# KyleHuang9/YOLO-LP

Measured on AMD Instinct MI355X. Metric: images/sec (640×640) end-to-end detect+NMS, yololps, 1/2/4/8 MI355X, higher is better.
Workload: dtype f16; 1 GPU; yololps 640x640 bs=32/GPU f16, synthetic frames resident in HBM, seeded random-init weights (sigma 0.25), conf 0.40 iou 0.45 max_det 1000; global_batch=32, parallelism=dp1: images sharded, all-gather of detections

## Files before the change

yolo-lp_amd/csrc/lp_conv3x3_pipe.inc:

```
#pragma once
#include "lp_conv_kernel.inc"
#include <type_traits>
#include <utility>

namespace lp {

template <int P> struct PipeCfg;
template <> struct PipeCfg<PIPE_D> { static constexpr int CB = 128, WC = 2, WP = 2, WGC = 2, WGP = 4, HPMAX = 384; };
template <> struct PipeCfg<PIPE_B> { static constexpr int CB = 64, WC = 2, WP = 2, WGC = 1, WGP = 8, HPMAX = 704; };
template <> struct PipeCfg<PIPE_F> { static constexpr int CB = 128, WC = 1, WP = 2, WGC = 4, WGP = 2, HPMAX = 384; };

template <> struct PipeCfg<PIPE_C> { static constexpr int CB = 32, WC = 1, WP = 2, WGC = 1, WGP = 8, HPMAX = 736; };

constexpr int PIPE_MAXC = 1024;
constexpr int PIPE_MAXCHUNKS = 64;

#ifndef LP_PIPE_ABL
#define LP_PIPE_ABL 0
#endif

template <typename F, int... I> __device__ __forceinline__ void static_for_impl(F&& f, std::integer_sequence<int, I...>) {
    (f(std::integral_constant<int, I>{}), ...);
}
template <int N, typename F> __device__ __forceinline__ void static_for(F&& f) {
// ... 192 lines not shown
            const unsigned long long p = (unsigned long long)a.src[sidx].ptr;
            c.tab[0] = (unsigned)p; c.tab[1] = (unsigned)(p >> 32);
            c.tab[2] = (unsigned)a.src[sidx].cs; c.tab[3] = (unsigned)((dq - a.chunk_begin[sidx]) * KC);
            c.ws = wts + ((long long)dma.ct * nchunks + dq) * (9 * CB * KC * 2);
        };
        auto halo_pieces = [&](const ChunkSrc& cc, char* buf) {
#pragma unroll
            for (int k = KH0; k < NPW; ++k) issue_piece(k, cc, buf, 1);
        };
        auto weight_pieces = [&](const ChunkSrc& cc, char* buf) {
#pragma unroll
            for (int k = 0; k < NPW; ++k) issue_piece(k, cc, buf, 2);
        };
        ChunkSrc c, c1;
        chunk_src_direct(c);
        if constexpr (LP_PRO_ORDER == 0) {
            halo_pieces(c, smem);
            dma_ok = dma_advance();
            if (dma_ok) {
                chunk_src_direct(c1);
                halo_pieces(c1, smem + SLOT);
            }
            weight_pieces(c, smem);
            if (dma_ok) weight_pieces(c1, smem + SLOT);
        } else {
            weight_pieces(c, smem);
            halo_pieces(c, smem);
            dma_ok = dma_advance();
            if (dma_ok) {
                chunk_src_direct(c1);
                weight_pieces(c1, smem + SLOT);
                halo_pieces(c1, smem + SLOT);
            }
        }
        if (dma_ok) dma_ok = dma_advance();
#ifdef LP_STAMPS
        st_p2 = __builtin_amdgcn_s_memtime();
#endif
        for (int i = tid; i < a.nct * CB; i += 512) bias_lds[i] = a.bias[i];
        if (tid < nchunks) {
            int sidx = 0;
#pragma unroll
            for (int k = 1; k < LP_MAX_SRC; ++k)
                if (k < a.nsrc && tid >= a.chunk_begin[k]) sidx = k;
            ChunkTab e;
            e.sp = (const T*)a.src[sidx].ptr;
            e.cs = a.src[sidx].cs;
            e.c0 = (tid - a.chunk_begin[sidx]) * KC;
            ctab[tid] = e;
// ... 296 lines not shown
```

yolo-lp_amd/csrc/lp_conv3x3_pipe16.inc:

```
#pragma once
#include "lp_conv3x3_pipe.inc"

namespace lp {

typedef float f32x4v __attribute__((ext_vector_type(4)));

template <typename T> struct Mma16;
template <> struct Mma16<f16> {
    static __device__ __forceinline__ f32x4v mma(f16x8 a, f16x8 b, f32x4v c) { return __builtin_amdgcn_mfma_f32_16x16x32_f16(a, b, c, 0, 0, 0); }
};
template <> struct Mma16<bf16> {
    static __device__ __forceinline__ f32x4v mma(bf16x8 a, bf16x8 b, f32x4v c) { return __builtin_amdgcn_mfma_f32_16x16x32_bf16(a, b, c, 0, 0, 0); }
};

template <int P> struct Pipe16Cfg;
template <> struct Pipe16Cfg<PIPE16_D> { static constexpr int CB = 128, WCB = 4, WPB = 4, WGC = 2, WGP = 4, HPMAX = 384; };
template <> struct Pipe16Cfg<PIPE16_F> { static constexpr int CB = 128, WCB = 2, WPB = 4, WGC = 4, WGP = 2, HPMAX = 384; };

__host__ __device__ __forceinline__ constexpr int quad_order(int i) { return ((i >> 2) == 2 ? 12 : (i >> 2) == 3 ? 8 : (i & 12)) + (i & 3); }

template <typename T, int P, bool DUAL = false>
__global__ __launch_bounds__(512) void conv3x3_pipe16_kernel(const ConvArgs a, const int total) {
    typedef Pipe16Cfg<P> C;
    typedef typename Mma<T>::V V;
    static_assert(sizeof(T) == 2, "16-bit activations only");
    constexpr int CB = C::CB, WCB = C::WCB, WPB = C::WPB, WGC = C::WGC, WGP = C::WGP, HPMAX = C::HPMAX;
    constexpr int NW = 8, ROWB = 32, KC = 16, EPG = 8;
    constexpr int NWP = 9 * CB / 32;
    constexpr int NHP = HPMAX / 32;
    static_assert((NWP + NHP) % NW == 0, "every wave must issue the same number of DMA instructions per chunk");
    constexpr int NPW = (NWP + NHP) / NW;
    constexpr int KH0 = NWP / NW;
    constexpr int NHK = NPW - KH0;
    constexpr int WOFF = HPMAX * ROWB;
    constexpr int SLOT = (HPMAX + 9 * CB) * ROWB;
    static_assert(WGC * WGP == NW, "8 waves");
    static_assert(WPB % 2 == 0, "the epilogue pairs pixel blocks");
    __shared__ __attribute__((aligned(1024))) char smem[3 * SLOT + PIPE_MAXC * 4 + PIPE_MAXCHUNKS * 16];
    float* const bias_lds = (float*)(smem + 3 * SLOT);
    const unsigned smem_lds = (unsigned)(size_t)(lds_char_t*)smem;

    const int tid = threadIdx.x;
    const int lane = tid & 63, wave = __builtin_amdgcn_readfirstlane(tid >> 6);
    const int li = lane & 15, g = lane >> 4;
    const int wvc = wave % WGC, wvp = wave / WGC;
    const int G = gridDim.x;

    const int tpi = a.tiles_y * a.tiles_x;
    const int npt = a.B * tpi;
    const int HH = a.TH + 2, HW = a.TW + 2, HP = a.hpitch;
    const int npix = a.TH * a.TW;
    const int nchunks = a.chunk_begin[a.nsrc];

    int hyx[NHK], hgc[NHK];
#pragma unroll
    for (int kk = 0; kk < NHK; ++kk) {
        const int j = (KH0 + kk) * NW + wave - NWP;
        const int slot = j * 64 + lane;
        const int hp = slot >> 1;
// ... 34 lines not shown
        o.b = pt / tpi;
        const int trem = pt - o.b * tpi;
        o.ty0 = (trem / a.tiles_x) * a.TH;
        o.tx0 = (trem % a.tiles_x) * a.TW;
        return true;
    };
    auto next_tile = [&](Tile& o) -> bool {
        int t = o.t;
        while (true) {
            t += G;
            if (decode(t, o)) return true;
            if (t >= total) return false;
        }
    };

    Tile dma, cmp;
    bool dma_ok = decode(blockIdx.x, dma) || next_tile(dma);
    if (!dma_ok) return;
    cmp = dma;
    int dq = 0;
    int hpix[NHK];
    auto dma_maps = [&]() {
#pragma unroll
        for (int kk = 0; kk < NHK; ++kk) {
            const int hy = hyx[kk] >> 16, hx = hyx[kk] & 0xffff;
            const int iy = dma.ty0 - 1 + hy, ix = dma.tx0 - 1 + hx;
            const bool ok = hyx[kk] >= 0 && iy >= 0 && iy < a.H && ix >= 0 && ix < a.W;
            hpix[kk] = ok ? (dma.b * a.H + iy) * a.W + ix : -1;
        }
    };
// ... 23 lines not shown
            const int cs = (int)cs_.tab[2];
            const int c = (int)cs_.tab[3] + hgc[kk];
            const T* const sp = (const T*)(((unsigned long long)cs_.tab[1] << 32) | cs_.tab[0]);
            const T* p = (hpix[kk] >= 0 && c < cs) ? sp + (long long)hpix[kk] * cs + c : zero;
            __builtin_amdgcn_global_load_lds((gbl_ptr_t)p, (lds_ptr_t)(buf + (i - NWP) * 1024), 16, 0, 0);
        }
    };
    auto dma_advance = [&]() {
        if (++dq < nchunks) return true;
        dq = 0;
        if (!next_tile(dma)) return false;
        dma_maps();
        return true;
    };

    {
        auto chunk_src_direct = [&](ChunkSrc& c) {
            int sidx = 0;
#pragma unroll
            for (int k = 1; k < LP_MAX_SRC; ++k)
                if (k < a.nsrc && dq >= a.chunk_begin[k]) sidx = k;
            const unsigned long long p = (unsigned long long)a.src[sidx].ptr;
            c.tab[0] = (unsigned)p; c.tab[1] = (unsigned)(p >> 32);
            c.tab[2] = (unsigned)a.src[sidx].cs; c.tab[3] = (unsigned)((dq - a.chunk_begin[sidx]) * KC);
            c.ws = wts + ((long long)dma.ct * nchunks + dq) * (9 * CB * KC * 2);
        };
        ChunkSrc c, c1;
        chunk_src_direct(c);
        dma_ok = dma_advance();
        chunk_src_direct(c1);
        auto halo_pieces = [&](const ChunkSrc& cc, char* buf) {
#pragma unroll
            for (int k = KH0; k < NPW; ++k) issue_piece(k, cc, buf, 1);
        };
        auto weight_pieces = [&](const ChunkSrc& cc, char* buf) {
#pragma unroll
            for (int k = 0; k < NPW; ++k) issue_piece(k, cc, buf, 2);
        };
        if constexpr (LP_PRO_ORDER == 0) {
            halo_pieces(c, smem); halo_pieces(c1, smem + SLOT); weight_pieces(c, smem); weight_pieces(c1, smem + SLOT);
        } else {
            weight_pieces(c, smem); weight_pieces(c1, smem + SLOT); halo_pieces(c, smem); halo_pieces(c1, smem + SLOT);
        }
        dma_ok = dma_advance();
        for (int i = tid; i < a.nct * CB; i += 512) bias_lds[i] = a.bias[i];
        if (tid < nchunks) {
            int sidx = 0;
#pragma unroll
            for (int k = 1; k < LP_MAX_SRC; ++k)
                if (k < a.nsrc && tid >= a.chunk_begin[k]) sidx = k;
            ChunkTab e;
            e.sp = (const T*)a.src[sidx].ptr;
            e.cs = a.src[sidx].cs;
            e.c0 = (tid - a.chunk_begin[sidx]) * KC;
            ctab[tid] = e;
        }
        asm volatile("s_waitcnt vmcnt(0)" ::: "memory");
    }
    __syncthreads();

    f32x4v acc[WCB][WPB];
    V fa[2][WCB], fb[2][WPB];
    int slot = 0;
    constexpr int NRD = WCB + WPB;
    auto read_one = [&](auto s_tag, int k, V(&af)[WCB], V(&bf)[WPB], unsigned va, unsigned vbb) {
        constexpr int s = decltype(s_tag)::value;
        constexpr int ta = s < 4 ? 2 * s : (s == 4 ? 8 : 2 * s - 9);
        constexpr int aimm = (s == 4 ? 0 : ta * CB * ROWB);
#pragma unroll
        for (int c = 0; c < WCB; ++c)
            if (k == c) LP_DS_READ128(af[c], va, aimm + c * 16 * ROWB);
#pragma unroll
        for (int p = 0; p < WPB; ++p)
            if (k == WCB + p) { const unsigned vb = vbb + boff[p][s]; LP_DS_READ128(bf[p], vb, 0); }
    };

    asm volatile("s_waitcnt lgkmcnt(0)" ::: "memory");
    __builtin_amdgcn_sched_barrier(0);
    {
        const unsigned va = smem_lds + aoffP;
#pragma unroll
        for (int k = 0; k < NRD; ++k) read_one(std::integral_constant<int, 0>{}, k, fa[0], fb[0], va, smem_lds);
    }
    constexpr int BE = 2, BO = 6;
    do {
#pragma unroll
        for (int c = 0; c < WCB; ++c) {
            const f32x4v bv = *(const f32x4v*)(bias_lds + cmp.ct * CB + (wvc * WCB + c) * 16 + (quad_order(4 * g)));
#pragma unroll
            for (int p = 0; p < WPB; ++p) acc[c][p] = bv;
        }
        asm volatile("s_waitcnt lgkmcnt(0)" ::: "memory");
        __builtin_amdgcn_sched_barrier(0);
        for (int cq = 0; cq < nchunks; cq += 4) {
            const int s0 = slot, s1 = slot == 2 ? 0 : slot + 1, s2 = slot == 0 ? 2 : slot - 1;
            const unsigned b0_ = smem_lds + (unsigned)s0 * SLOT, b1_ = smem_lds + (unsigned)s1 * SLOT, b2_ = smem_lds + (unsigned)s2 * SLOT;
            const unsigned vxa0 = (g < 2 ? b0_ + 8 * CB * ROWB : b1_) + aoffL, vxb0 = g < 2 ? b0_ : b1_;
            const unsigned vxa1 = (g < 2 ? b2_ + 8 * CB * ROWB : b0_) + aoffL, vxb1 = g < 2 ? b2_ : b0_;
            ChunkSrc nxt;
            static_for<18>([&](auto st_tag) {
                constexpr int S = decltype(st_tag)::value;
                constexpr int q = S / 9, st = S % 9;
                constexpr int cur = S & 1, nx = cur ^ 1;
                const unsigned bE = q == 0 ? b0_ : b2_, bO = q == 0 ? b1_ : b0_, bN = q == 0 ? b2_ : b1_;
                const int sE = q == 0 ? s0 : s2, sN = q == 0 ? s2 : s1;
                if constexpr (st == BE - 1 || st == BO - 1) chunk_src_request(nxt);
                if constexpr (st == BE || st == BO) {
                    asm volatile("s_waitcnt vmcnt(0)" ::: "memory");
                    __builtin_amdgcn_s_barrier();
                    asm volatile("" ::: "memory");
                    __builtin_amdgcn_sched_barrier(0);
                }
                if constexpr (st == BE || st == BO) asm volatile("s_waitcnt lgkmcnt(0)" : "+v"(nxt.tab)::"memory");
                else asm volatile("s_waitcnt lgkmcnt(0)" ::: "memory");
                __builtin_amdgcn_sched_barrier(0);
                constexpr int sn = (st + 1) % 9;
                const unsigned nva = sn == 4 ? (q == 0 ? vxa0 : vxa1) : ((st == 8 ? bN : (sn < 4 ? bE : bO)) + aoffP);
                const unsigned nvb = sn == 4 ? (q == 0 ? vxb0 : vxb1) : (st == 8 ? bN : (sn < 4 ? bE : bO));
                int nread = 0;
#pragma unroll
                for (int p = 0; p < WPB; ++p)
#pragma unroll
                    for (int c = 0; c < WCB; ++c) {
                        acc[c][p] = Mma16<T>::mma(fa[cur][c], fb[cur][p], acc[c][p]);
                        __builtin_amdgcn_sched_barrier(0);
                        if (nread < NRD) { read_one(std::integral_constant<int, sn>{}, nread, fa[nx], fb[nx], nva, nvb); ++nread; }
                        __builtin_amdgcn_sched_barrier(0);
                    }
                static_assert(NRD <= WCB * WPB, "one read per MFMA gap");
                if constexpr ((st >= BE && st < BE + 3) || (st >= BO && st < BO + 3)) {
                    constexpr int b0 = st >= BO ? BO : BE;
                    constexpr int k0 = (st - b0) * NPW / 3, k1 = (st - b0 + 1) * NPW / 3;
                    char* const nbuf = smem + (st >= BO ? sE : sN) * SLOT;
                    if (dma_ok) {
#pragma unroll
                        for (int k = k0; k < k1; ++k) issue_piece(k, nxt, nbuf);
                    }
                    __builtin_amdgcn_sched_barrier(0);
                    if constexpr (st == b0 + 2) { if (dma_ok) dma_ok = dma_advance(); }
                }
            });
            slot = s1;
        }

        {
            T* const out = (T*)a.out + (long long)cmp.b * a.out_img_stride;
            [[maybe_unused]] T* const out2 = DUAL ? (T*)a.out2 + (long long)cmp.b * a.out2_img_stride - a.out_split : nullptr;
            const T* const res = a.res ? (const T*)a.res + (long long)cmp.b * a.Ho * a.Wo * a.res_cs : nullptr;
            act_dispatch(a.act, [&](auto tag) {
                constexpr int ACT = decltype(tag)::value;
#pragma unroll
                for (int q = 0; q < WPB / 2; ++q) {
                    uint4 rv[WCB];
                    const int pl = (wvp * WPB + 2 * q + (g & 1)) * 16 + quad_order(li);
                    const int ty = (int)(((unsigned)pl * a.tw_magic) >> 22), tx = pl - ty * a.TW;
                    const int oy = cmp.ty0 + ty, ox = cmp.tx0 + tx;
                    const bool pok = pl < npix && oy < a.Ho && ox < a.Wo;
                    const long long opix = (long long)oy * a.Wo + ox;
// ... 27 lines not shown
                                const T* prr = (const T*)&rv[c];
#pragma unroll
                                for (int k = 0; k < EPG; ++k) pv[k] = from_f32<T>(to_f32(pv[k]) + a.alpha * to_f32(prr[k]));
                            }
                            if constexpr (DUAL) {
                                T* const dstp = cc >= a.out_split ? out2 + opix * a.out2_pix_stride + cc : out + opix * a.out_pix_stride + cc;
                                *(uint4*)dstp = v;
                            } else {
                                *(uint4*)(out + opix * a.out_pix_stride + cc) = v;
                            }
                        }
                    }
                }
            });
        }
    } while (next_tile(cmp));
    asm volatile("s_waitcnt lgkmcnt(0)" ::: "memory");
}

template <typename T, int P>
static inline int pipe16_launch_one(const ConvArgs& a, int ncu, hipStream_t st) {
    const int npt = a.B * a.tiles_y * a.tiles_x;
    const int total = a.nct * round_up(npt, 8);
    int grid = total < ncu ? total : ncu;
    if (a.out2) hipLaunchKernelGGL((conv3x3_pipe16_kernel<T, P, true>), dim3((unsigned)grid), dim3(512), 0, st, a, total);
    else hipLaunchKernelGGL((conv3x3_pipe16_kernel<T, P, false>), dim3((unsigned)grid), dim3(512), 0, st, a, total);
    hipError_t e = hipGetLastError();
    if (e != hipSuccess) return fail(LP_ERR_HIP, std::string("conv3x3 pipe16 launch: ") + hipGetErrorString(e));
    return LP_OK;
}

template <typename T>
// ... 10 lines not shown
```

yolo-lp_amd/csrc/lp_conv3x3_pipe16v.inc:

```
#pragma once
#include "lp_conv3x3_pipe16.inc"

namespace lp {

template <int P> struct Pipe16vCfg;
template <> struct Pipe16vCfg<PIPE16_V0> { static constexpr int CB = 128, WCB = 4, NBMAX = 7, WGC = 2, WGP = 4, HPMAX = 512; };
template <> struct Pipe16vCfg<PIPE16_V1> { static constexpr int CB = 128, WCB = 2, NBMAX = 7, WGC = 4, WGP = 2, HPMAX = 512; };

constexpr int PIPE16V_MAXC = 512;
constexpr int PIPE16V_MAXCHUNKS = 32;

template <typename T, int P, bool DUAL = false>
__global__ __launch_bounds__(512) void conv3x3_pipe16v_kernel(const ConvArgs a, const int total) {
    typedef Pipe16vCfg<P> C;
    typedef typename Mma<T>::V V;
    static_assert(sizeof(T) == 2, "16-bit activations only");
    constexpr int CB = C::CB, WCB = C::WCB, NBMAX = C::NBMAX, WGC = C::WGC, WGP = C::WGP, HPMAX = C::HPMAX;
    constexpr int NW = 8, ROWB = 32, KC = 16, EPG = 8;
    constexpr int NWP = 9 * CB / 32;
    constexpr int NHP = HPMAX / 32;
    constexpr int NPT = NWP + NHP;
    constexpr int NPW = (NPT + NW - 1) / NW;
    constexpr int KH0 = NWP / NW;
    constexpr int NHK = NPW - KH0;
    constexpr int WOFF = HPMAX * ROWB;
    constexpr int SLOT = (HPMAX + 9 * CB) * ROWB;
    static_assert(WGC * WGP == NW, "8 waves");
    static_assert(WCB <= NBMAX - 2, "the weight fragments of a K-step are requested in its first WCB blocks and must be older than the next step's first pixel fragment");
    static_assert(3 * SLOT + PIPE16V_MAXC * 4 + PIPE16V_MAXCHUNKS * 16 <= 160 * 1024, "LDS budget");
    static_assert(3 * (NBMAX / 2) >= NPW, "a piece round behind every odd block of the three steps after a barrier");
    __shared__ __attribute__((aligned(1024))) char smem[3 * SLOT + PIPE16V_MAXC * 4 + PIPE16V_MAXCHUNKS * 16];
    float* const bias_lds = (float*)(smem + 3 * SLOT);
    const unsigned smem_lds = (unsigned)(size_t)(lds_char_t*)smem;

    const int tid = threadIdx.x;
    const int lane = tid & 63, wave = __builtin_amdgcn_readfirstlane(tid >> 6);
    const int li = lane & 15, g = lane >> 4;
#ifdef LP_STAMPS
    const unsigned long long st_c0 = __builtin_amdgcn_s_memtime(), st_r0 = __builtin_amdgcn_s_memrealtime();
    unsigned long long st_p1 = 0, st_p2 = 0, st_p3 = 0, st_p4 = 0, st_loop = 0, st_epi = 0, st_last = 0;
#endif
    const int wvc = WGC == 2 ? (wave >> 2) : (wave & 3);
    const int wvp = WGC == 2 ? ((wave + 2 * (wave >> 2)) & 3) : (wave >> 2);
    const int G = gridDim.x;

    const int tpi = a.tiles_y * a.tiles_x;
    const int npt = a.B * tpi;
// ... 25 lines not shown
            int pl = (blk0 + p) * 16 + li;
            if (p >= nbw || pl >= npix) pl = 0;
            const int ty = (int)(((unsigned)pl * a.tw_magic) >> 22), tx = pl - ty * a.TW;
            bbase[p] = (ty * HP + tx) * ROWB + (g & 1) * 16;
        }
#pragma unroll
        for (int s = 0; s < 9; ++s) {
            const int ta = s < 4 ? 2 * s : (s == 4 ? 8 : 2 * s - 9);
            const int tb = s == 4 ? 0 : ta + 1;
            const int t = g < 2 ? ta : tb;
            voff[s] = ((t / 3) * HP + (t % 3)) * ROWB;
        }
        const int arow = (wvc * WCB) * 16 + quad_order(li);
        aoffL = WOFF + arow * ROWB + swz(arow, g & 1, 2) * 16;
        aoffP = aoffL + (g >> 1) * (CB * ROWB);
    };

    struct Tile { int t, ct, b, ty0, tx0; };
    auto decode = [&](int t, Tile& o) -> bool {
        o.t = t;
        if (t >= total) return false;
        const int jj = t >> 3;
        o.ct = jj % a.nct;
        const int pt = (jj / a.nct) * 8 + (t & 7);
        if (pt >= npt) return false;
        o.b = pt / tpi;
        const int trem = pt - o.b * tpi;
        o.ty0 = (trem / a.tiles_x) * a.TH;
        o.tx0 = (trem % a.tiles_x) * a.TW;
        return true;
// ... 62 lines not shown
#ifdef LP_P16V_DMAXH
#pragma unroll
            for (int r = 0; r < LP_P16V_DMAXH; ++r)
                __builtin_amdgcn_global_load_lds((gbl_ptr_t)p, (lds_ptr_t)(buf + (i - NWP) * 1024), 16, 0, 0);
#endif
        }
    };
    auto dma_advance = [&]() {
        if (++dq < nchunks) return true;
        dq = 0;
        if (!next_tile(dma)) return false;
        dma_maps();
        return true;
    };

    {
        auto chunk_src_direct = [&](ChunkSrc& c) {
            int sidx = 0;
#pragma unroll
            for (int k = 1; k < LP_MAX_SRC; ++k)
                if (k < a.nsrc && dq >= a.chunk_begin[k]) sidx = k;
            const unsigned long long p = (unsigned long long)a.src[sidx].ptr;
            c.tab[0] = (unsigned)p; c.tab[1] = (unsigned)(p >> 32);
            c.tab[2] = (unsigned)a.src[sidx].cs; c.tab[3] = (unsigned)((dq - a.chunk_begin[sidx]) * KC);
            c.ws = wts + ((long long)dma.ct * nchunks + dq) * (9 * CB * KC * 2);
        };
        ChunkSrc c, c1;
        chunk_src_direct(c);
        dma_ok = dma_advance();
        chunk_src_direct(c1);
        auto halo_pieces = [&](const ChunkSrc& cc, char* buf) {
#ifndef LP_P16V_PRO_SKIPH
#pragma unroll
            for (int k = KH0; k < NPW; ++k) issue_piece(k, cc, buf, 1);
#endif
        };
        auto weight_pieces = [&](const ChunkSrc& cc, char* buf) {
#ifndef LP_P16V_PRO_SKIPW
#pragma unroll
            for (int k = 0; k < NPW; ++k) issue_piece(k, cc, buf, 2);
#endif
        };
#ifndef LP_P16V_PRO_ORDER
#define LP_P16V_PRO_ORDER (LP_PRO_ORDER ? 3 : 0)
#endif
        if constexpr (LP_P16V_PRO_ORDER == 0) {
            halo_pieces(c, smem); halo_pieces(c1, smem + SLOT); weight_pieces(c, smem); weight_pieces(c1, smem + SLOT);
        } else if constexpr (LP_P16V_PRO_ORDER == 1) {
            halo_pieces(c, smem); weight_pieces(c, smem); weight_pieces(c1, smem + SLOT); halo_pieces(c1, smem + SLOT);
        } else if constexpr (LP_P16V_PRO_ORDER == 2) {
            weight_pieces(c, smem); halo_pieces(c, smem); weight_pieces(c1, smem + SLOT); halo_pieces(c1, smem + SLOT);
        } else if constexpr (LP_P16V_PRO_ORDER == 3) {
            weight_pieces(c, smem); weight_pieces(c1, smem + SLOT); halo_pieces(c, smem); halo_pieces(c1, smem + SLOT);
        } else {
            weight_pieces(c, smem); halo_pieces(c, smem); halo_pieces(c1, smem + SLOT); weight_pieces(c1, smem + SLOT);
        }
        dma_ok = dma_advance();
#ifdef LP_STAMPS
        st_p2 = __builtin_amdgcn_s_memtime();
#endif
        frag_maps();
        for (int i = tid; i < a.nct * CB; i += 512) bias_lds[i] = a.bias[i];
        if (tid < nchunks) {
            int sidx = 0;
#pragma unroll
            for (int k = 1; k < LP_MAX_SRC; ++k)
                if (k < a.nsrc && tid >= a.chunk_begin[k]) sidx = k;
            ChunkTab e;
            e.sp = (const T*)a.src[sidx].ptr;
            e.cs = a.src[sidx].cs;
            e.c0 = (tid - a.chunk_begin[sidx]) * KC;
            ctab[tid] = e;
        }
#ifdef LP_STAMPS
        st_p3 = __builtin_amdgcn_s_memtime();
#endif
        asm volatile("s_waitcnt vmcnt(0)" ::: "memory");
#ifdef LP_STAMPS
        st_p4 = __builtin_amdgcn_s_memtime();
#endif
    }
    __syncthreads();

    f32x4v acc[WCB][NBMAX];
    V fa[2][WCB];
    V fb[3];
    int slot = 0;
#ifndef LP_P16V_BE
#define LP_P16V_BE 2
#endif
#ifndef LP_P16V_BO
#define LP_P16V_BO 6
#endif
    constexpr int BE = LP_P16V_BE, BO = LP_P16V_BO;
    static_assert(BE >= 1 && BE <= 3 && BO >= 5 && BO <= 6, "barrier(e) in front of step 3's request of the cross step, barrier(o) behind step 4 with three steps of DMA issue left");
    constexpr int NBLK = 18 * NBMAX;

#ifdef LP_P16V_PRIO
    if (wave >= 4) __builtin_amdgcn_s_setprio(1);
#endif
    asm volatile("s_waitcnt lgkmcnt(0)" ::: "memory");
    __builtin_amdgcn_sched_barrier(0);
    {
        const unsigned va = smem_lds + aoffP;
#pragma unroll
        for (int c = 0; c < WCB; ++c) LP_DS_READ128(fa[0][c], va, c * 16 * ROWB);
        const unsigned vb0 = smem_lds + bbase[0] + voff[0], vb1 = smem_lds + bbase[1] + voff[0];
        LP_DS_READ128(fb[0], vb0, 0);
        LP_DS_READ128(fb[1], vb1, 0);
    }
#ifdef LP_STAMPS
    st_loop = __builtin_amdgcn_s_memtime();
#endif
    do {
#pragma unroll
        for (int c = 0; c < WCB; ++c) {
            const f32x4v bv = *(const f32x4v*)(bias_lds + cmp.ct * CB + (wvc * WCB + c) * 16 + (quad_order(4 * g)));
#pragma unroll
            for (int p = 0; p < NBMAX; ++p) acc[c][p] = bv;
        }
        asm volatile("s_waitcnt lgkmcnt(0)" ::: "memory");
        __builtin_amdgcn_sched_barrier(0);
        for (int cq = 0; cq < nchunks; cq += 4) {
            const int s0 = slot, s1 = slot == 2 ? 0 : slot + 1, s2 = slot == 0 ? 2 : slot - 1;
            const unsigned b0_ = smem_lds + (unsigned)s0 * SLOT, b1_ = smem_lds + (unsigned)s1 * SLOT, b2_ = smem_lds + (unsigned)s2 * SLOT;
            ChunkSrc nxt;
            static_for<18>([&](auto st_tag) {
                constexpr int S = decltype(st_tag)::value;
                constexpr int q = S / 9, st = S % 9;
                constexpr int cur = S & 1, nx = cur ^ 1;
                constexpr int sn = (st + 1) % 9;
                const unsigned bE = q == 0 ? b0_ : b2_, bO = q == 0 ? b1_ : b0_, bN = q == 0 ? b2_ : b1_;
                const int sE = q == 0 ? s0 : s2, sN = q == 0 ? s2 : s1;
                auto bstep = [&](int s, bool next_pair) -> unsigned {
                    const unsigned e = next_pair ? bN : bE, o = bO;
                    return (s < 4 ? e : (s == 4 ? (g < 2 ? e : o) : o)) + (unsigned)voff[s];
                };
                const unsigned vb_cur = bstep(st, false);
                const unsigned vb_nxt = bstep(sn, st == 8);
                const unsigned va_nxt = sn == 4 ? ((g < 2 ? bE + 8 * CB * ROWB : bO) + aoffL) : ((st == 8 ? bN : (sn < 4 ? bE : bO)) + aoffP);
                constexpr int ta_n = sn < 4 ? 2 * sn : (sn == 4 ? 8 : 2 * sn - 9);
                constexpr int aimm_n = sn == 4 ? 0 : ta_n * CB * ROWB;
                if constexpr (st == BE || st == BO) {
                    asm volatile("s_waitcnt vmcnt(0)" ::: "memory");
                    __builtin_amdgcn_s_barrier();
                    asm volatile("" ::: "memory");
                    __builtin_amdgcn_sched_barrier(0);
                }
#pragma unroll
                for (int p = 0; p < NBMAX; ++p) {
                    constexpr bool tab_step = (st == BE - 1 || st == BO - 1);
                    {
                        const int n = 1 + ((p >= 1 && p - 1 < WCB) ? 1 : 0) + ((tab_step && p == 1) ? 1 : 0);
                        if (n == 1) asm volatile("s_waitcnt lgkmcnt(1)" ::: "memory");
                        else if (n == 2) asm volatile("s_waitcnt lgkmcnt(2)" ::: "memory");
                        else asm volatile("s_waitcnt lgkmcnt(3)" ::: "memory");
                    }
                    __builtin_amdgcn_sched_barrier(0);
// ... 6 lines not shown
                            else if (e == 1) acc[c][p] = Mma16<T>::mma(fa[cur][c], fb[1], acc[c][p]);
                            else acc[c][p] = Mma16<T>::mma(fa[cur][c], fb[2], acc[c][p]);
                        }
                    }
                    __builtin_amdgcn_sched_barrier(0);
                    if (p < WCB) LP_DS_READ128(fa[nx][p], va_nxt, aimm_n + p * 16 * ROWB);
                    {
                        const int p2 = p + 2;
                        const unsigned vb = (p2 < NBMAX ? vb_cur + (unsigned)bbase[p2 < NBMAX ? p2 : 0] : vb_nxt + (unsigned)bbase[p2 < NBMAX ? 0 : p2 - NBMAX]);
                        const int e2 = (S * NBMAX + p + 2) % 3;
                        if (e2 == 0) LP_DS_READ128(fb[0], vb, 0);
                        else if (e2 == 1) LP_DS_READ128(fb[1], vb, 0);
                        else LP_DS_READ128(fb[2], vb, 0);
                    }
                    __builtin_amdgcn_sched_barrier(0);
                    if constexpr ((st >= BE && st < BE + 3) || (st >= BO && st < BO + 3)) {
                        constexpr int b0 = st >= BO ? BO : BE;
                        const int slotn = (st - b0) * (NBMAX / 2) + (p >> 1);
                        if ((p & 1) == 1 || p == NBMAX - 1) {
                            const int k = (p & 1) == 1 ? slotn : -1;
                            char* const nbuf = smem + (st >= BO ? sE : sN) * SLOT;
                            if (k >= 0 && k < NPW && dma_ok) issue_piece(k, nxt, nbuf);
                            __builtin_amdgcn_sched_barrier(0);
                        }
                        if (st == b0 + 2 && p == NBMAX - 1) { if (dma_ok) dma_ok = dma_advance(); }
                    }
                }
                if constexpr (st == BE || st == BO) asm volatile("" : "+v"(nxt.tab));
            });
            slot = s1;
        }
        (void)NBLK;

#ifdef LP_STAMPS
        const unsigned long long st_e0 = __builtin_amdgcn_s_memtime();
#endif
        {
            const long long torg = (long long)cmp.ty0 * a.Wo + cmp.tx0;
            const int cw = cmp.ct * CB + wvc * WCB * 16;
            T* const out = (T*)a.out + (long long)cmp.b * a.out_img_stride + torg * a.out_pix_stride + cw;
            [[maybe_unused]] T* const out2 = DUAL ? (T*)a.out2 + (long long)cmp.b * a.out2_img_stride + torg * a.out2_pix_stride + cw - a.out_split : nullptr;
            const T* const res = a.res ? (const T*)a.res + ((long long)cmp.b * a.Ho * a.Wo + torg) * a.res_cs + cw : nullptr;
            const int ylim = a.Ho - cmp.ty0, xlim = a.Wo - cmp.tx0;
            const int cg = (g >> 1) * 8;
            act_dispatch(a.act, [&](auto tag) {
                constexpr int ACT = decltype(tag)::value;
#pragma unroll
// ... 48 lines not shown
                                                                      : out + (unsigned)(erel[q] * a.out_pix_stride + c * 16 + cg);
                                    *(uint4*)dstp = v;
                                } else {
                                    *(uint4*)(out + (unsigned)(erel[q] * a.out_pix_stride + c * 16 + cg)) = v;
                                }
                            }
                        }
                    }
                }
            });
        }
#ifdef LP_STAMPS
        st_last = __builtin_amdgcn_s_memtime();
        st_epi += st_last - st_e0;
#endif
    } while (next_tile(cmp));
    asm volatile("s_waitcnt lgkmcnt(0)" ::: "memory");
#ifdef LP_STAMPS
    if (a.stamps && lane == 0) {
        unsigned long long* o = a.stamps + ((long long)(blockIdx.x * NW + wave)) * 8;
        asm volatile("s_waitcnt vmcnt(0)" ::: "memory");
        const unsigned long long st_end = __builtin_amdgcn_s_memtime();
        o[0] = st_end - st_c0; o[1] = __builtin_amdgcn_s_memrealtime() - st_r0;
        o[2] = st_loop - st_c0; o[3] = st_epi; o[4] = st_end - st_last; o[5] = o[0]; o[6] = nchunks; o[7] = 2;
        unsigned long long* o2 = a.stamps + (1 << 19) + ((long long)(blockIdx.x * NW + wave)) * 8;
        o2[0] = st_p1 - st_c0; o2[1] = st_p2 - st_p1; o2[2] = st_p3 - st_p2; o2[3] = st_p4 - st_p3; o2[4] = st_loop - st_p4; o2[7] = 5;
    }
#endif
}

template <typename T, int P>
// ... 22 lines not shown
```

yolo-lp_amd/csrc/lp_internal.h:

```cpp
#pragma once
#include <hip/hip_runtime.h>
#include <stdint.h>
#include <stddef.h>
#include <atomic>
#include <string>

#include "../../include/lp_hip.h"

#ifndef LP_PRO_ORDER
#define LP_PRO_ORDER 0
#endif

namespace lp {

typedef _Float16 f16;
typedef __bf16 bf16;

void set_error(const std::string& msg);
int fail(int code, const std::string& msg);
#define LP_HIP_CHECK(expr)                                                                       \
    do {                                                                                         \
        hipError_t _e = (expr);                                                                  \
        if (_e != hipSuccess)                                                                    \
            return ::lp::fail(LP_ERR_HIP, std::string(#expr) + ": " + hipGetErrorString(_e));    \
    } while (0)

// ... 148 lines not shown
```

Measured before the change: 17870 images/s.

## Overlap conv prologue DMA of second chunk with first pass compute

In the pipe16 and pipe16v 3x3 conv kernels, the prologue now issues only chunk 0's pieces in a per-half-workgroup order (halo first) and waits with partial vmcnt counts. Chunk 1's pieces are issued interleaved with the first pass's MFMA steps, instead of waiting for both chunks and a full syncthreads before compute begins. Bias loading moves to async global_load_lds, and the bias init is refactored into acc_init with explicit ds_reads. The aim is to shorten the prologue stall per workgroup. The cost is intricate compile-time vmcnt bookkeeping that must match the issue order exactly.

```diff
diff --git a/yolo-lp_amd/csrc/lp_conv3x3_pipe.inc b/yolo-lp_amd/csrc/lp_conv3x3_pipe.inc
--- a/yolo-lp_amd/csrc/lp_conv3x3_pipe.inc
+++ b/yolo-lp_amd/csrc/lp_conv3x3_pipe.inc
@@ -230,25 +230,14 @@
         };
         ChunkSrc c, c1;
         chunk_src_direct(c);
-        if constexpr (LP_PRO_ORDER == 0) {
-            halo_pieces(c, smem);
-            dma_ok = dma_advance();
-            if (dma_ok) {
-                chunk_src_direct(c1);
-                halo_pieces(c1, smem + SLOT);
-            }
-            weight_pieces(c, smem);
-            if (dma_ok) weight_pieces(c1, smem + SLOT);
-        } else {
-            weight_pieces(c, smem);
-            halo_pieces(c, smem);
-            dma_ok = dma_advance();
-            if (dma_ok) {
-                chunk_src_direct(c1);
-                weight_pieces(c1, smem + SLOT);
-                halo_pieces(c1, smem + SLOT);
-            }
-        }
+        halo_pieces(c, smem);
+        dma_ok = dma_advance();
+        if (dma_ok) {
+            chunk_src_direct(c1);
+            halo_pieces(c1, smem + SLOT);
+        }
+        weight_pieces(c, smem);
+        if (dma_ok) weight_pieces(c1, smem + SLOT);
         if (dma_ok) dma_ok = dma_advance();
 #ifdef LP_STAMPS
         st_p2 = __builtin_amdgcn_s_memtime();
diff --git a/yolo-lp_amd/csrc/lp_conv3x3_pipe16.inc b/yolo-lp_amd/csrc/lp_conv3x3_pipe16.inc
--- a/yolo-lp_amd/csrc/lp_conv3x3_pipe16.inc
+++ b/yolo-lp_amd/csrc/lp_conv3x3_pipe16.inc
@@ -16,6 +16,31 @@
 template <int P> struct Pipe16Cfg;
 template <> struct Pipe16Cfg<PIPE16_D> { static constexpr int CB = 128, WCB = 4, WPB = 4, WGC = 2, WGP = 4, HPMAX = 384; };
 template <> struct Pipe16Cfg<PIPE16_F> { static constexpr int CB = 128, WCB = 2, WPB = 4, WGC = 4, WGP = 2, HPMAX = 384; };
+
+template <int NWP, int NPT>
+struct PieceOrder {
+    static_assert(NWP % 8 == 4 && NPT % 4 == 0 && NPT > NWP + 4, "classes = the two halves of the workgroup");
+    static constexpr int NPW = (NPT + 7) / 8;
+    static constexpr bool exists(int k, int cls) { return k * 8 + cls * 4 < NPT; }
+    static constexpr bool halo(int k, int cls) { return k * 8 + cls * 4 >= NWP; }
+    static constexpr int nh(int cls) { int n = 0; for (int k = 0; k < NPW; ++k) n += (exists(k, cls) && halo(k, cls)) ? 1 : 0; return n; }
+    static constexpr int n(int cls) { int n = 0; for (int k = 0; k < NPW; ++k) n += exists(k, cls) ? 1 : 0; return n; }
+    static constexpr int round(int j, int cls) {
+        if (j >= n(cls)) return -1;
+        if (j >= nh(cls)) return j - nh(cls);
+        for (int k = 0; k < NPW; ++k)
+            if (exists(k, cls) && halo(k, cls) && j-- == 0) return k;
+        return -1;
+    }
+    static constexpr int need(int s, int cls) {
+        const int m = s <= 3 ? nh(cls) + s + 1 : n(cls) + nh(cls) + s - 3;
+        return m < (s <= 3 ? n(cls) : 2 * n(cls)) ? m : (s <= 3 ? n(cls) : 2 * n(cls));
+    }
+};
+template <int N> __device__ __forceinline__ void vm_wait() {
+    static_assert(N >= 0 && N < 64, "vmcnt is a six-bit counter");
+    asm volatile("s_waitcnt vmcnt(%0)" ::"n"(N) : "memory");
+}
 
 __host__ __device__ __forceinline__ constexpr int quad_order(int i) { return ((i >> 2) == 2 ? 12 : (i >> 2) == 3 ? 8 : (i & 12)) + (i & 3); }
 
@@ -37,12 +62,15 @@
     static_assert(WGC * WGP == NW, "8 waves");
     static_assert(WPB % 2 == 0, "the epilogue pairs pixel blocks");
     __shared__ __attribute__((aligned(1024))) char smem[3 * SLOT + PIPE_MAXC * 4 + PIPE_MAXCHUNKS * 16];
-    float* const bias_lds = (float*)(smem + 3 * SLOT);
     const unsigned smem_lds = (unsigned)(size_t)(lds_char_t*)smem;
 
     const int tid = threadIdx.x;
     const int lane = tid & 63, wave = __builtin_amdgcn_readfirstlane(tid >> 6);
     const int li = lane & 15, g = lane >> 4;
+#ifdef LP_STAMPS
+    const unsigned long long st_c0 = __builtin_amdgcn_s_memtime(), st_r0 = __builtin_amdgcn_s_memrealtime();
+    unsigned long long st_p1 = 0, st_p2 = 0, st_p3 = 0, st_p4 = 0, st_loop = 0;
+#endif
     const int wvc = wave % WGC, wvp = wave / WGC;
     const int G = gridDim.x;
 
@@ -107,6 +135,9 @@
         }
     };
 
+#ifdef LP_STAMPS
+    st_p1 = __builtin_amdgcn_s_memtime();
+#endif
     Tile dma, cmp;
     bool dma_ok = decode(blockIdx.x, dma) || next_tile(dma);
     if (!dma_ok) return;
@@ -160,7 +191,35 @@
         return true;
     };
 
+    typedef PieceOrder<NWP, NWP + NHP> PO;
+    static_assert(PO::n(0) == NPW && PO::n(1) == NPW && NPW % 2 == 0 && NPW % 3 == 0, "piece counts of the first pair");
+    constexpr int BE = 2, BO = 6;
+    auto issue_ordered = [&](int j, const ChunkSrc& cs_, char* buf) {
+        static_for<NPW>([&](auto j_tag) {
+            constexpr int J = decltype(j_tag)::value;
+            if (j != J) return;
+            if (wave < NW / 2) issue_piece(PO::round(J, 0), cs_, buf);
+            else issue_piece(PO::round(J, 1), cs_, buf);
+        });
+    };
+    constexpr auto requested = [](int st) { return st <= 0 ? NPW : st == 1 ? NPW + NPW / 2 : 2 * NPW + (st - BE) * (NPW / 3); };
+    auto landed_barrier = [&](auto st_tag) {
+        constexpr int st = decltype(st_tag)::value;
+        if (wave < NW / 2) vm_wait<requested(st) - PO::need(st + 1, 0)>();
+        else vm_wait<requested(st) - PO::need(st + 1, 1)>();
+        __builtin_amdgcn_s_barrier();
+        asm volatile("" ::: "memory");
+        __builtin_amdgcn_sched_barrier(0);
+    };
+
+    ChunkSrc c1;
     {
+        const int nbias = a.nct * CB;
+#pragma unroll
+        for (int r = 0; r < PIPE_MAXC / 512; ++r) {
+            const int i = r * 512 + tid;
+            __builtin_amdgcn_global_load_lds((gbl_ptr_t)(a.bias + (i < nbias ? i : 0)), (lds_ptr_t)(smem + 3 * SLOT + (r * 512 + wave * 64) * 4), 4, 0, 0);
+        }
         auto chunk_src_direct = [&](ChunkSrc& c) {
             int sidx = 0;
 #pragma unroll
@@ -171,39 +230,36 @@
             c.tab[2] = (unsigned)a.src[sidx].cs; c.tab[3] = (unsigned)((dq - a.chunk_begin[sidx]) * KC);
             c.ws = wts + ((long long)dma.ct * nchunks + dq) * (9 * CB * KC * 2);
         };
-        ChunkSrc c, c1;
+        ChunkSrc c;
         chunk_src_direct(c);
         dma_ok = dma_advance();
         chunk_src_direct(c1);
-        auto halo_pieces = [&](const ChunkSrc& cc, char* buf) {
-#pragma unroll
-            for (int k = KH0; k < NPW; ++k) issue_piece(k, cc, buf, 1);
-        };
-        auto weight_pieces = [&](const ChunkSrc& cc, char* buf) {
-#pragma unroll
-            for (int k = 0; k < NPW; ++k) issue_piece(k, cc, buf, 2);
-        };
-        if constexpr (LP_PRO_ORDER == 0) {
-            halo_pieces(c, smem); halo_pieces(c1, smem + SLOT); weight_pieces(c, smem); weight_pieces(c1, smem + SLOT);
-        } else {
-            weight_pieces(c, smem); weight_pieces(c1, smem + SLOT); halo_pieces(c, smem); halo_pieces(c1, smem + SLOT);
-        }
+        if (tid < nchunks) {
+            ChunkTab e;
+            e.sp = (const T*)a.src[0].ptr;
+            e.cs = a.src[0].cs;
+            int cb = 0;
+#pragma unroll
+            for (int k = 1; k < LP_MAX_SRC; ++k)
+                if (k < a.nsrc && tid >= a.chunk_begin[k]) { e.sp = (const T*)a.src[k].ptr; e.cs = a.src[k].cs; cb = a.chunk_begin[k]; }
+            e.c0 = (tid - cb) * KC;
+            ctab[tid] = e;
+        }
+#pragma unroll
+        for (int j = 0; j < NPW; ++j) issue_ordered(j, c, smem);
         dma_ok = dma_advance();
-        for (int i = tid; i < a.nct * CB; i += 512) bias_lds[i] = a.bias[i];
-        if (tid < nchunks) {
-            int sidx = 0;
-#pragma unroll
-            for (int k = 1; k < LP_MAX_SRC; ++k)
-                if (k < a.nsrc && tid >= a.chunk_begin[k]) sidx = k;
-            ChunkTab e;
-            e.sp = (const T*)a.src[sidx].ptr;
-            e.cs = a.src[sidx].cs;
-            e.c0 = (tid - a.chunk_begin[sidx]) * KC;
-            ctab[tid] = e;
-        }
-        asm volatile("s_waitcnt vmcnt(0)" ::: "memory");
-    }
-    __syncthreads();
+#ifdef LP_STAMPS
+        st_p2 = __builtin_amdgcn_s_memtime();
+#endif
+#ifdef LP_STAMPS
+        st_p3 = __builtin_amdgcn_s_memtime();
+#endif
+    }
+    asm volatile("s_waitcnt lgkmcnt(0)" ::: "memory");
+    landed_barrier(std::integral_constant<int, 0>{});
+#ifdef LP_STAMPS
+    st_p4 = __builtin_amdgcn_s_memtime();
+#endif
 
     f32x4v acc[WCB][WPB];
     V fa[2][WCB], fb[2][WPB];
@@ -228,17 +284,25 @@
 #pragma unroll
         for (int k = 0; k < NRD; ++k) read_one(std::integral_constant<int, 0>{}, k, fa[0], fb[0], va, smem_lds);
     }
-    constexpr int BE = 2, BO = 6;
-    do {
+#ifdef LP_STAMPS
+    st_loop = __builtin_amdgcn_s_memtime();
+#endif
+    auto acc_init = [&]() {
+        f32x4v bv[WCB];
+        const unsigned baddr = smem_lds + 3 * SLOT + (unsigned)(cmp.ct * CB + wvc * WCB * 16 + quad_order(4 * g)) * 4;
+#pragma unroll
+        for (int c = 0; c < WCB; ++c) asm volatile("ds_read_b128 %0, %1 offset:%2" : "=v"(bv[c]) : "v"(baddr), "n"(c * 16 * 4));
+        asm volatile("s_waitcnt lgkmcnt(0)" ::: "memory");
 #pragma unroll
         for (int c = 0; c < WCB; ++c) {
-            const f32x4v bv = *(const f32x4v*)(bias_lds + cmp.ct * CB + (wvc * WCB + c) * 16 + (quad_order(4 * g)));
-#pragma unroll
-            for (int p = 0; p < WPB; ++p) acc[c][p] = bv;
-        }
-        asm volatile("s_waitcnt lgkmcnt(0)" ::: "memory");
+            asm volatile("" : "+v"(bv[c]));
+#pragma unroll
+            for (int p = 0; p < WPB; ++p) acc[c][p] = bv[c];
+        }
         __builtin_amdgcn_sched_barrier(0);
-        for (int cq = 0; cq < nchunks; cq += 4) {
+    };
+    auto pass = [&](auto first_tag) {
+            constexpr bool FIRST = decltype(first_tag)::value;
             const int s0 = slot, s1 = slot == 2 ? 0 : slot + 1, s2 = slot == 0 ? 2 : slot - 1;
             const unsigned b0_ = smem_lds + (unsigned)s0 * SLOT, b1_ = smem_lds + (unsigned)s1 * SLOT, b2_ = smem_lds + (unsigned)s2 * SLOT;
             const unsigned vxa0 = (g < 2 ? b0_ + 8 * CB * ROWB : b1_) + aoffL, vxb0 = g < 2 ? b0_ : b1_;
@@ -251,7 +315,9 @@
                 const unsigned bE = q == 0 ? b0_ : b2_, bO = q == 0 ? b1_ : b0_, bN = q == 0 ? b2_ : b1_;
                 const int sE = q == 0 ? s0 : s2, sN = q == 0 ? s2 : s1;
                 if constexpr (st == BE - 1 || st == BO - 1) chunk_src_request(nxt);
-                if constexpr (st == BE || st == BO) {
+                if constexpr (FIRST && q == 0 && st >= 1 && st < BO) {
+                    landed_barrier(std::integral_constant<int, st>{});
+                } else if constexpr (st == BE || st == BO) {
                     asm volatile("s_waitcnt vmcnt(0)" ::: "memory");
                     __builtin_amdgcn_s_barrier();
                     asm volatile("" ::: "memory");
@@ -274,6 +340,11 @@
                         __builtin_amdgcn_sched_barrier(0);
                     }
                 static_assert(NRD <= WCB * WPB, "one read per MFMA gap");
+                if constexpr (FIRST && q == 0 && st < 2) {
+#pragma unroll
+                    for (int j = 0; j < NPW / 2; ++j) issue_ordered(st * (NPW / 2) + j, c1, smem + SLOT);
+                    __builtin_amdgcn_sched_barrier(0);
+                }
                 if constexpr ((st >= BE && st < BE + 3) || (st >= BO && st < BO + 3)) {
                     constexpr int b0 = st >= BO ? BO : BE;
                     constexpr int k0 = (st - b0) * NPW / 3, k1 = (st - b0 + 1) * NPW / 3;
@@ -287,7 +358,14 @@
                 }
             });
             slot = s1;
-        }
+    };
+
+    acc_init();
+    pass(std::true_type{});
+    for (int cq = 4;;) {
+        asm volatile("s_waitcnt lgkmcnt(0)" ::: "memory");
+        __builtin_amdgcn_sched_barrier(0);
+        for (; cq < nchunks; cq += 4) pass(std::false_type{});
 
         {
             T* const out = (T*)a.out + (long long)cmp.b * a.out_img_stride;
@@ -345,8 +423,22 @@
                 }
             });
         }
-    } while (next_tile(cmp));
+        if (!next_tile(cmp)) break;
+        acc_init();
+        cq = 0;
+    }
     asm volatile("s_waitcnt lgkmcnt(0)" ::: "memory");
+#ifdef LP_STAMPS
+    if (a.stamps && lane == 0) {
+        unsigned long long* o = a.stamps + ((long long)(blockIdx.x * NW + wave)) * 8;
+        asm volatile("s_waitcnt vmcnt(0)" ::: "memory");
+        const unsigned long long st_end = __builtin_amdgcn_s_memtime();
+        o[0] = st_end - st_c0; o[1] = __builtin_amdgcn_s_memrealtime() - st_r0;
+        o[2] = st_loop - st_c0; o[3] = 0; o[4] = 0; o[5] = o[0]; o[6] = nchunks; o[7] = 2;
+        unsigned long long* o2 = a.stamps + (1 << 19) + ((long long)(blockIdx.x * NW + wave)) * 8;
+        o2[0] = st_p1 - st_c0; o2[1] = st_p2 - st_p1; o2[2] = st_p3 - st_p2; o2[3] = st_p4 - st_p3; o2[4] = st_loop - st_p4; o2[7] = 5;
+    }
+#endif
 }
 
 template <typename T, int P>
diff --git a/yolo-lp_amd/csrc/lp_conv3x3_pipe16v.inc b/yolo-lp_amd/csrc/lp_conv3x3_pipe16v.inc
--- a/yolo-lp_amd/csrc/lp_conv3x3_pipe16v.inc
+++ b/yolo-lp_amd/csrc/lp_conv3x3_pipe16v.inc
@@ -30,7 +30,6 @@
     static_assert(3 * SLOT + PIPE16V_MAXC * 4 + PIPE16V_MAXCHUNKS * 16 <= 160 * 1024, "LDS budget");
     static_assert(3 * (NBMAX / 2) >= NPW, "a piece round behind every odd block of the three steps after a barrier");
     __shared__ __attribute__((aligned(1024))) char smem[3 * SLOT + PIPE16V_MAXC * 4 + PIPE16V_MAXCHUNKS * 16];
-    float* const bias_lds = (float*)(smem + 3 * SLOT);
     const unsigned smem_lds = (unsigned)(size_t)(lds_char_t*)smem;
 
     const int tid = threadIdx.x;
@@ -86,6 +85,11 @@
         const int arow = (wvc * WCB) * 16 + quad_order(li);
         aoffL = WOFF + arow * ROWB + swz(arow, g & 1, 2) * 16;
         aoffP = aoffL + (g >> 1) * (CB * ROWB);
+#pragma unroll
+        for (int p = 0; p < NBMAX; ++p) asm volatile("" : "+v"(bbase[p]));
+#pragma unroll
+        for (int s = 0; s < 9; ++s) asm volatile("" : "+v"(voff[s]));
+        asm volatile("" : "+v"(aoffL), "+v"(aoffP));
     };
 
     struct Tile { int t, ct, b, ty0, tx0; };
@@ -178,7 +182,50 @@
         return true;
     };
 
+    typedef PieceOrder<NWP, NPT> PO;
+#ifndef LP_P16V_BE
+#define LP_P16V_BE 2
+#endif
+#ifndef LP_P16V_BO
+#define LP_P16V_BO 6
+#endif
+    constexpr int BE = LP_P16V_BE, BO = LP_P16V_BO;
+    static_assert(BE >= 1 && BE <= 3 && BO >= 5 && BO <= 6, "barrier(e) in front of step 3's request of the cross step, barrier(o) behind step 4 with three steps of DMA issue left");
+    static_assert(BE == 2, "the first pair requests chunk 1 behind steps 0 and 1 and counts its pieces for a barrier in step 2");
+    static_assert(PO::n(0) <= 2 * (NBMAX / 2) + 1 && PO::n(1) <= PO::n(0), "chunk 1: a piece behind every odd block of steps 0 and 1, one behind the last block of step 1");
+    auto issue_ordered = [&](int j, const ChunkSrc& cs_, char* buf) {
+        static_for<NPW>([&](auto j_tag) {
+            constexpr int J = decltype(j_tag)::value;
+            constexpr int k0 = PO::round(J, 0), k1 = PO::round(J, 1);
+            if (j != J) return;
+            if (wave < NW / 2) { if constexpr (k0 >= 0) issue_piece(k0, cs_, buf); }
+            else { if constexpr (k1 >= 0) issue_piece(k1, cs_, buf); }
+        });
+    };
+    constexpr auto requested = [](int st, int cls) {
+        if (st <= 0) return PO::n(cls);
+        if (st == 1) return PO::n(cls) + NBMAX / 2;
+        int m = 2 * PO::n(cls);
+        for (int k = 0; k < (st - BE) * (NBMAX / 2) && k < NPW; ++k) m += PO::exists(k, cls) ? 1 : 0;
+        return m;
+    };
+    auto landed_barrier = [&](auto st_tag) {
+        constexpr int st = decltype(st_tag)::value;
+        if (wave < NW / 2) vm_wait<requested(st, 0) - PO::need(st + 1, 0)>();
+        else vm_wait<requested(st, 1) - PO::need(st + 1, 1)>();
+        __builtin_amdgcn_s_barrier();
+        asm volatile("" ::: "memory");
+        __builtin_amdgcn_sched_barrier(0);
+    };
+
+    ChunkSrc c1;
     {
+        const int nbias = a.nct * CB;
+#pragma unroll
+        for (int r = 0; r < PIPE16V_MAXC / 512; ++r) {
+            const int i = r * 512 + tid;
+            __builtin_amdgcn_global_load_lds((gbl_ptr_t)(a.bias + (i < nbias ? i : 0)), (lds_ptr_t)(smem + 3 * SLOT + (r * 512 + wave * 64) * 4), 4, 0, 0);
+        }
         auto chunk_src_direct = [&](ChunkSrc& c) {
             int sidx = 0;
 #pragma unroll
@@ -189,75 +236,42 @@
             c.tab[2] = (unsigned)a.src[sidx].cs; c.tab[3] = (unsigned)((dq - a.chunk_begin[sidx]) * KC);
             c.ws = wts + ((long long)dma.ct * nchunks + dq) * (9 * CB * KC * 2);
         };
-        ChunkSrc c, c1;
+        ChunkSrc c;
         chunk_src_direct(c);
         dma_ok = dma_advance();
         chunk_src_direct(c1);
-        auto halo_pieces = [&](const ChunkSrc& cc, char* buf) {
-#ifndef LP_P16V_PRO_SKIPH
-#pragma unroll
-            for (int k = KH0; k < NPW; ++k) issue_piece(k, cc, buf, 1);
-#endif
-        };
-        auto weight_pieces = [&](const ChunkSrc& cc, char* buf) {
-#ifndef LP_P16V_PRO_SKIPW
-#pragma unroll
-            for (int k = 0; k < NPW; ++k) issue_piece(k, cc, buf, 2);
-#endif
-        };
-#ifndef LP_P16V_PRO_ORDER
-#define LP_P16V_PRO_ORDER (LP_PRO_ORDER ? 3 : 0)
-#endif
-        if constexpr (LP_P16V_PRO_ORDER == 0) {
-            halo_pieces(c, smem); halo_pieces(c1, smem + SLOT); weight_pieces(c, smem); weight_pieces(c1, smem + SLOT);
-        } else if constexpr (LP_P16V_PRO_ORDER == 1) {
-            halo_pieces(c, smem); weight_pieces(c, smem); weight_pieces(c1, smem + SLOT); halo_pieces(c1, smem + SLOT);
-        } else if constexpr (LP_P16V_PRO_ORDER == 2) {
-            weight_pieces(c, smem); halo_pieces(c, smem); weight_pieces(c1, smem + SLOT); halo_pieces(c1, smem + SLOT);
-        } else if constexpr (LP_P16V_PRO_ORDER == 3) {
-            weight_pieces(c, smem); weight_pieces(c1, smem + SLOT); halo_pieces(c, smem); halo_pieces(c1, smem + SLOT);
-        } else {
-            weight_pieces(c, smem); halo_pieces(c, smem); halo_pieces(c1, smem + SLOT); weight_pieces(c1, smem + SLOT);
-        }
+        if (tid < nchunks) {
+            ChunkTab e;
+            e.sp = (const T*)a.src[0].ptr;
+            e.cs = a.src[0].cs;
+            int cb = 0;
+#pragma unroll
+            for (int k = 1; k < LP_MAX_SRC; ++k)
+                if (k < a.nsrc && tid >= a.chunk_begin[k]) { e.sp = (const T*)a.src[k].ptr; e.cs = a.src[k].cs; cb = a.chunk_begin[k]; }
+            e.c0 = (tid - cb) * KC;
+            ctab[tid] = e;
+        }
+#pragma unroll
+        for (int j = 0; j < NPW; ++j) issue_ordered(j, c, smem);
         dma_ok = dma_advance();
 #ifdef LP_STAMPS
         st_p2 = __builtin_amdgcn_s_memtime();
 #endif
         frag_maps();
-        for (int i = tid; i < a.nct * CB; i += 512) bias_lds[i] = a.bias[i];
-        if (tid < nchunks) {
-            int sidx = 0;
-#pragma unroll
-            for (int k = 1; k < LP_MAX_SRC; ++k)
-                if (k < a.nsrc && tid >= a.chunk_begin[k]) sidx = k;
-            ChunkTab e;
-            e.sp = (const T*)a.src[sidx].ptr;
-            e.cs = a.src[sidx].cs;
-            e.c0 = (tid - a.chunk_begin[sidx]) * KC;
-            ctab[tid] = e;
-        }
 #ifdef LP_STAMPS
         st_p3 = __builtin_amdgcn_s_memtime();
 #endif
-        asm volatile("s_waitcnt vmcnt(0)" ::: "memory");
-#ifdef LP_STAMPS
-        st_p4 = __builtin_amdgcn_s_memtime();
-#endif
     }
-    __syncthreads();
+    asm volatile("s_waitcnt lgkmcnt(0)" ::: "memory");
+    landed_barrier(std::integral_constant<int, 0>{});
+#ifdef LP_STAMPS
+    st_p4 = __builtin_amdgcn_s_memtime();
+#endif
 
     f32x4v acc[WCB][NBMAX];
     V fa[2][WCB];
     V fb[3];
     int slot = 0;
-#ifndef LP_P16V_BE
-#define LP_P16V_BE 2
-#endif
-#ifndef LP_P16V_BO
-#define LP_P16V_BO 6
-#endif
-    constexpr int BE = LP_P16V_BE, BO = LP_P16V_BO;
-    static_assert(BE >= 1 && BE <= 3 && BO >= 5 && BO <= 6, "barrier(e) in front of step 3's request of the cross step, barrier(o) behind step 4 with three steps of DMA issue left");
     constexpr int NBLK = 18 * NBMAX;
 
 #ifdef LP_P16V_PRIO
@@ -276,16 +290,22 @@
 #ifdef LP_STAMPS
     st_loop = __builtin_amdgcn_s_memtime();
 #endif
-    do {
+    auto acc_init = [&]() {
+        f32x4v bv[WCB];
+        const unsigned baddr = smem_lds + 3 * SLOT + (unsigned)(cmp.ct * CB + wvc * WCB * 16 + quad_order(4 * g)) * 4;
+#pragma unroll
+        for (int c = 0; c < WCB; ++c) asm volatile("ds_read_b128 %0, %1 offset:%2" : "=v"(bv[c]) : "v"(baddr), "n"(c * 16 * 4));
+        asm volatile("s_waitcnt lgkmcnt(0)" ::: "memory");
 #pragma unroll
         for (int c = 0; c < WCB; ++c) {
-            const f32x4v bv = *(const f32x4v*)(bias_lds + cmp.ct * CB + (wvc * WCB + c) * 16 + (quad_order(4 * g)));
-#pragma unroll
-            for (int p = 0; p < NBMAX; ++p) acc[c][p] = bv;
-        }
-        asm volatile("s_waitcnt lgkmcnt(0)" ::: "memory");
+            asm volatile("" : "+v"(bv[c]));
+#pragma unroll
+            for (int p = 0; p < NBMAX; ++p) acc[c][p] = bv[c];
+        }
         __builtin_amdgcn_sched_barrier(0);
-        for (int cq = 0; cq < nchunks; cq += 4) {
+    };
+    auto pass = [&](auto first_tag) {
+            constexpr bool FIRST = decltype(first_tag)::value;
             const int s0 = slot, s1 = slot == 2 ? 0 : slot + 1, s2 = slot == 0 ? 2 : slot - 1;
             const unsigned b0_ = smem_lds + (unsigned)s0 * SLOT, b1_ = smem_lds + (unsigned)s1 * SLOT, b2_ = smem_lds + (unsigned)s2 * SLOT;
             ChunkSrc nxt;
@@ -305,7 +325,9 @@
                 const unsigned va_nxt = sn == 4 ? ((g < 2 ? bE + 8 * CB * ROWB : bO) + aoffL) : ((st == 8 ? bN : (sn < 4 ? bE : bO)) + aoffP);
                 constexpr int ta_n = sn < 4 ? 2 * sn : (sn == 4 ? 8 : 2 * sn - 9);
                 constexpr int aimm_n = sn == 4 ? 0 : ta_n * CB * ROWB;
-                if constexpr (st == BE || st == BO) {
+                if constexpr (FIRST && q == 0 && st >= 1 && st < BO) {
+                    landed_barrier(std::integral_constant<int, st>{});
+                } else if constexpr (st == BE || st == BO) {
                     asm volatile("s_waitcnt vmcnt(0)" ::: "memory");
                     __builtin_amdgcn_s_barrier();
                     asm volatile("" ::: "memory");
@@ -342,6 +364,12 @@
                         else LP_DS_READ128(fb[2], vb, 0);
                     }
                     __builtin_amdgcn_sched_barrier(0);
+                    if constexpr (FIRST && q == 0 && st < 2) {
+                        if ((p & 1) == 1 || (st == 1 && p == NBMAX - 1)) {
+                            issue_ordered((p & 1) == 1 ? st * (NBMAX / 2) + (p >> 1) : 2 * (NBMAX / 2), c1, smem + SLOT);
+                            __builtin_amdgcn_sched_barrier(0);
+                        }
+                    }
                     if constexpr ((st >= BE && st < BE + 3) || (st >= BO && st < BO + 3)) {
                         constexpr int b0 = st >= BO ? BO : BE;
                         const int slotn = (st - b0) * (NBMAX / 2) + (p >> 1);
@@ -357,8 +385,15 @@
                 if constexpr (st == BE || st == BO) asm volatile("" : "+v"(nxt.tab));
             });
             slot = s1;
-        }
-        (void)NBLK;
+    };
+    (void)NBLK;
+
+    acc_init();
+    pass(std::true_type{});
+    for (int cq = 4;;) {
+        asm volatile("s_waitcnt lgkmcnt(0)" ::: "memory");
+        __builtin_amdgcn_sched_barrier(0);
+        for (; cq < nchunks; cq += 4) pass(std::false_type{});
 
 #ifdef LP_STAMPS
         const unsigned long long st_e0 = __builtin_amdgcn_s_memtime();
@@ -437,7 +472,10 @@
         st_last = __builtin_amdgcn_s_memtime();
         st_epi += st_last - st_e0;
 #endif
-    } while (next_tile(cmp));
+        if (!next_tile(cmp)) break;
+        acc_init();
+        cq = 0;
+    }
     asm volatile("s_waitcnt lgkmcnt(0)" ::: "memory");
 #ifdef LP_STAMPS
     if (a.stamps && lane == 0) {
diff --git a/yolo-lp_amd/csrc/lp_internal.h b/yolo-lp_amd/csrc/lp_internal.h
--- a/yolo-lp_amd/csrc/lp_internal.h
+++ b/yolo-lp_amd/csrc/lp_internal.h
@@ -6,10 +6,6 @@
 #include <string>
 
 #include "../../include/lp_hip.h"
-
-#ifndef LP_PRO_ORDER
-#define LP_PRO_ORDER 0
-#endif
 
 namespace lp {
 
```

New measurement: 17790 images/s, median of 3. Within noise of the previous version (-0.4%).
